# lgemc/WildlifeMapper

Measured on AMD Instinct MI355X. Metric: 1024x1024 tiles/sec (whole node), higher is better.
Workload: dtype fp16; 1 GPU; vit_h full path fft+encoder+decoder+PostProcess/NMS, fp16 MFMA, batch=16 tiles/GPU of 1024x1024x3 (BASELINE.json configs[2]); parallelism=dp1 tile shard, weights=seed 0 synthetic (random init), tolerance=logits within 1e-3 relative of the fp32 CPU forward, identical NMS index lists

## Files before the change

wildlifemapper_amd/csrc/dec_kernels.h:

```cpp
#pragma once
#include "wm_common.h"
#include "../../include/wm_hip.h"

namespace wm {

template <int HD, int QB, int NW = 1>
__global__ __launch_bounds__(64 * NW) void mha32_kernel(const float* __restrict__ q, const float* __restrict__ k,
                                                   const float* __restrict__ v, float* __restrict__ out,
                                                   int nq, int nk, int heads) {
    const int lane = threadIdx.x & 63, wave = threadIdx.x >> 6;
    const int q0 = blockIdx.x * QB, head = blockIdx.y, b = blockIdx.z;
    const int C = heads * HD;
    const float scale = 1.0f / sqrtf((float)HD);
    float qv[QB][HD], m[QB], l[QB], acc[QB][HD];
#pragma unroll
    for (int i = 0; i < QB; ++i) {
        const int qi = min(q0 + i, nq - 1);
        const float* qp = q + ((size_t)b * nq + qi) * C + head * HD;
#pragma unroll
        for (int d = 0; d < HD; d += 4) {
            const f32x4 t = *(const f32x4*)(qp + d);
            qv[i][d] = t[0]; qv[i][d + 1] = t[1]; qv[i][d + 2] = t[2]; qv[i][d + 3] = t[3];
        }
        m[i] = -1e30f; l[i] = 0.f;
#pragma unroll
        for (int d = 0; d < HD; ++d) acc[i][d] = 0.f;
    }
    for (int key = wave * 64 + lane; key < nk; key += 64 * NW) {
        const float* kp = k + ((size_t)b * nk + key) * C + head * HD;
        const float* vp = v + ((size_t)b * nk + key) * C + head * HD;
        float kr[HD], vr[HD];
#pragma unroll
        for (int d = 0; d < HD; d += 4) {
            const f32x4 t = *(const f32x4*)(kp + d);
// ... 269 lines not shown
            if (sscore[j] > score || (sscore[j] == score && j < i)) ++rank;
        }
    }
    if (cand) sorder[rank] = i;
    __syncthreads();
    int nms_rank = -1, kept = 0;
    for (int r = 0; r < ncand; ++r) {
        const int a = sorder[r];
        const bool alive = sdead[a] == 0;
        if (alive) {
            if (i == a) nms_rank = kept;
            ++kept;
            if (cand && rank > r && sdead[i] == 0) {
                const float xx0 = fmaxf(sx0[a], x0), yy0 = fmaxf(sy0[a], y0);
                const float xx1 = fminf(sx1[a], x1), yy1 = fminf(sy1[a], y1);
                const float iw = fmaxf(0.f, xx1 - xx0), ih = fmaxf(0.f, yy1 - yy0);
                const float inter = iw * ih;
                const float iou = inter / (sarea[a] + sarea[i] - inter);
                if (iou > iou_thr) sdead[i] = 1;
            }
        }
        __syncthreads();
    }
    if (live) {
        wm_box_record o;
        o.box[0] = x0; o.box[1] = y0; o.box[2] = x1; o.box[3] = y1;
        o.score = score; o.label = label;
        o.flags = (conf ? WM_FLAG_CONF : 0) | (cand ? WM_FLAG_SCORE : 0) | (nms_rank >= 0 ? WM_FLAG_NMS : 0);
        o.nms_rank = nms_rank;
        rec[(size_t)b * NQ + i] = o;
    }
}

__global__ __launch_bounds__(256) void add_bcast_kernel(const float* __restrict__ a, const float* __restrict__ b, float* __restrict__ out,
                                                        int64_t rows, int C, int mod) {
    const int64_t n4 = rows * C / 4;
    for (int64_t i = (int64_t)blockIdx.x * 256 + threadIdx.x; i < n4; i += (int64_t)gridDim.x * 256) {
        const int64_t r = (i * 4) / C;
        const int c = (int)((i * 4) % C);
        const f32x4 y = *(const f32x4*)(b + (r % mod) * C + c);
        *(f32x4*)(out + i * 4) = a ? *(const f32x4*)(a + i * 4) + y : y;
    }
}

}
```

wildlifemapper_amd/csrc/host_attn.h:

```cpp
#pragma once
#include "attn_glob4.h"
#include "attn_glob8.h"
#include "attn_window.h"
#include "dec_kernels.h"
#include "misc_kernels.h"
#include "host_core.h"

namespace {

struct AttnTimeline { const char* tag = nullptr; int waves = 0, marks = 0; };
template <auto KERN, class... Extra>
int launch_attn(wm_handle* h, hipStream_t s, int kclass, double flops, AttnTimeline tl, int grid, int block, int lds, const AttnArgs& a, Extra... extra) {
    lds += (tl.tag && WM_DEV_TIMELINE) ? 4096 : 0;
    WM_TRY(set_max_lds((const void*)KERN, lds));
    Bracket br(h, s, kclass, flops, 0.0);
    if (tl.tag) WM_DEV_HOOK((dev_attn_timeline<KERN>(tl.tag, tl.waves, tl.marks, dim3(grid), dim3(block), lds, s, a, extra...)));
    hipLaunchKernelGGL(KERN, dim3(grid), dim3(block), lds, s, a, extra...);
    HIP_TRY(hipGetLastError());
    return 0;
}

template <class T16, int HD, bool REL>
int launch_attn_global_t(wm_handle* h, hipStream_t s, const AttnArgs& a, int batch, int kclass) {
    static const bool four_wave = getenv("WM_ATTN_4WAVE") && atoi(getenv("WM_ATTN_4WAVE")) != 0;
    const double flops = 4.0 * batch * a.heads * (double)a.nq * a.nk * HD;
    if (a.nq % 256 == 0 && a.nk >= 128 && !four_wave)
        return launch_attn<attn_global8_kernel<T16, HD, REL>>(h, s, kclass, flops, {"g8", 8, 64}, (a.nq / 256) * a.heads * batch, 512, Global8Lds<HD, REL>::TOTAL, a);
    return launch_attn<attn_global_kernel<T16, HD, REL>>(h, s, kclass, flops, {}, (a.nq / 128) * a.heads * batch, 256, GlobalLds<HD, REL>::TOTAL, a);
}

template <class T16>
int launch_attn_global_p(wm_handle* h, hipStream_t s, const AttnArgs& a, int batch, int hd, bool rel, int kclass) {
    if (a.nq % 128 || a.nk % 64) return fail("attention: nq=%d nk=%d must be multiples of 128/64", a.nq, a.nk);
    if (rel && (a.nq != T || a.nk != T)) return fail("attention: rel-pos path needs 4096 queries and keys");
    auto none = [&] { return fail("attention: head_dim=%d rel=%d not built (64, 80, 128)", hd, (int)rel); };
    if (rel) return by_head_dim<64, 80>(hd, [&](auto d) { return launch_attn_global_t<T16, decltype(d)::value, true>(h, s, a, batch, kclass); }, none);
    return by_head_dim<64, 80, 128>(hd, [&](auto d) { return launch_attn_global_t<T16, decltype(d)::value, false>(h, s, a, batch, kclass); }, none);
}
int launch_attn_global(wm_handle* h, hipStream_t s, int prec, const AttnArgs& a, int batch, int hd, bool rel) {
// ... 51 lines not shown
    if (!x.q_prescaled) WM_TRY(scale_q_copy(s, prec, a, batch, D));
    if (window == 0) return launch_attn_global(h, s, prec, a, batch, hd, true);
    if (window != 14) return fail("attention: window=%d unsupported (14 or 0)", window);
    {
        uint16_t* b16 = nullptr;
        bool convert = true;
        if (h) {
            auto it = h->bias16.find({qkv_bias, prec});
            if (it != h->bias16.end()) { b16 = it->second; convert = false; }
            else { WM_TRY(dalloc(h, &b16, (size_t)3 * D * 2)); h->bias16[{qkv_bias, prec}] = b16; }
        } else {
            void* pb = nullptr;
            WM_TRY(op_scratch(s, 0, (size_t)3 * D * 2, &pb));
            b16 = (uint16_t*)pb;
        }
        if (convert) WM_TRY(launch_cvt_f32_to_16(s, prec, qkv_bias, b16, 3 * D / 4));
        a.qkv_bias16 = (const u16*)b16;
    }
    return by_head_dim<64, 80>(hd, [&](auto d) {
        return by_type16(prec, [&](auto t) { return launch_attn_window_t<decltype(t), decltype(d)::value>(h, s, a, batch); });
    }, [&] { return fail("attention: head_dim=%d not built for windows (64, 80)", hd); });
}

int launch_mha16(wm_handle* h, hipStream_t s, int prec, const void* q, int qs, const void* k, int ks, const void* v, int vs,
                 void* out, int os, int batch, int heads, int hd, int nq, int nk, int q_prescaled = 0) {
    AttnArgs a{};
    a.q = (const u16*)q; a.k = (const u16*)k; a.v = (const u16*)v; a.out = (u16*)out;
    a.q_stride = qs; a.k_stride = ks; a.v_stride = vs; a.out_stride = os;
    a.nq = nq; a.nk = nk; a.scale = 1.0f / sqrtf((float)hd); a.heads = heads;
    if (!q_prescaled) WM_TRY(scale_q_copy(s, prec, a, batch, heads * hd));
    return launch_attn_global(h, s, prec, a, batch, hd, false);
}

int launch_mha32(wm_handle* h, hipStream_t s, const float* q, const float* k, const float* v, float* out, int batch,
                 int heads, int hd, int nq, int nk) {
    Bracket br(h, s, WM_KCLASS_OTHER, 4.0 * batch * heads * (double)nq * nk * hd, 0.0);
    const bool share = nk >= 1024;
    constexpr int KC = 256;
    if (hd == 16 && nq <= 64 && nk >= 1024 && nk % KC == 0) {
        const int nchunk = nk / KC;
        const size_t need = (size_t)batch * heads * nchunk * 64 * (16 + 2) * 4;
        float* part = nullptr;
        if (h) {
            if (h->mha_part_cap < need) {
                if (h->mha_part) dfree(h, h->mha_part);
                h->mha_part = nullptr; h->mha_part_cap = 0;
                WM_TRY(dalloc(h, &h->mha_part, need));
                h->mha_part_cap = need;
            }
            part = h->mha_part;
        } else {
            void* pb = nullptr;
            WM_TRY(op_scratch(s, 1, need, &pb));
            part = (float*)pb;
        }
        hipLaunchKernelGGL((mha32_keysplit_kernel<16, KC>), dim3(nchunk, heads, batch), dim3(256), 0, s, q, k, v, part, nq, nk, heads);
        hipLaunchKernelGGL((mha32_merge_chunks_kernel<16>), dim3(heads, batch), dim3(64 * 4), 0, s, (const float*)part, out, nq, nchunk, heads);
    } else if (hd == 16 && nk == NQ && nq >= 1024)
        hipLaunchKernelGGL((mha32_fewkeys_kernel<16, NQ>), dim3((nq + 255) / 256, heads, batch), dim3(256), 0, s, q, k, v, out, nq, heads);
    else if (hd == 16 && share) hipLaunchKernelGGL((mha32_kernel<16, 4, 4>), dim3((nq + 3) / 4, heads, batch), dim3(256), 0, s, q, k, v, out, nq, nk, heads);
    else if (hd == 16) hipLaunchKernelGGL((mha32_kernel<16, 1>), dim3(nq, heads, batch), dim3(64), 0, s, q, k, v, out, nq, nk, heads);
    else if (hd == 32) hipLaunchKernelGGL((mha32_kernel<32, 1>), dim3(nq, heads, batch), dim3(64), 0, s, q, k, v, out, nq, nk, heads);
    else return fail("mha32: head_dim=%d not built (16, 32)", hd);
    HIP_TRY(hipGetLastError());
    return 0;
}

}
```

wildlifemapper_amd/csrc/host_core.h:

```cpp
#pragma once
#include <hip/hip_runtime.h>

#include <cmath>
#include <cstdarg>
#include <cstdio>
#include <cstdlib>
#include <cstring>
#include <atomic>
#include <map>
#include <tuple>
#include <type_traits>
#include <mutex>
#include <set>
#include <string>
#include <algorithm>
#include <array>
#include <vector>

#include "../../include/wm_hip.h"
#include "wm_common.h"

#ifndef WM_DEV_TIMELINE
#define WM_DEV_TIMELINE 0
#endif
// ... 125 lines not shown
    hipEvent_t a, b;
    int kclass;
    double flops, bytes;
};

struct Profiler {
    bool on = false;
    std::vector<EvPair> used;
    std::vector<std::pair<hipEvent_t, hipEvent_t>> pool;
    wm_kclass_stat acc[WM_KCLASS_COUNT] = {};
};

}

struct wm_handle {
    wm_config cfg{};
    int fp8_gemms = WM_FP8_ALL;
    int fp8_bf16_tail = 0, fp8_bf16_head = 0;
    int fp16_tail = 0;
    int device = 0;
    int D = 0, depth = 0, heads = 0, hd = 0, prec = 0, maxB = 0;
    bool is_global[64] = {};
    bool finalized = false, enc_ready = false, dec_ready = false;
    std::map<std::string, std::vector<int64_t>> expected;
    std::map<std::string, HostW> staged;
    std::map<std::string, uint16_t*> w16;
    std::map<std::string, uint16_t*> wfold;
    std::map<std::string, float*> fold_c1, fold_c2;
    std::map<std::string, float*> wsrc32;
    float* fold_stats = nullptr;
    uint16_t* lo16 = nullptr;
    bool split = false;
    bool rows8 = true;
    bool fold_from16 = false;
    int* overflow = nullptr;
    bool fold = false, fold_bf16 = false;
    std::map<std::string, uint16_t*> w16p;
    std::map<std::string, uint8_t*> w8k;
    std::map<std::string, uint8_t*> w8;
    uint8_t* ao8 = nullptr;
    std::map<std::string, float*> w32;
    std::vector<void*> allocs;
    Profiler prof;
    std::map<const float*, std::pair<uint16_t*, uint16_t*>> w32x3;
    std::map<std::pair<const float*, int>, uint16_t*> bias16;
    float* mha_part = nullptr;
    size_t mha_part_cap = 0;
    bool row_major = false;
    bool sat_on = false;
    unsigned long long* sat_counts = nullptr;
    int tap_which = -2;
    float* tap_buf = nullptr;

    float *resid = nullptr, *tokbase = nullptr;
    uint16_t *xn16 = nullptr, *ao16 = nullptr, *qkv16 = nullptr, *hid16 = nullptr;
    uint16_t *p16 = nullptr, *h16 = nullptr, *he16 = nullptr, *hp16 = nullptr, *pt16 = nullptr, *q16 = nullptr,
             *kv16 = nullptr, *aoh16 = nullptr, *y1n16 = nullptr, *h1_16 = nullptr, *y2_16 = nullptr, *y2t16 = nullptr;
    float *pt32 = nullptr, *y1 = nullptr, *y1n32 = nullptr, *z32 = nullptr;
    float *n1 = nullptr, *n2 = nullptr, *emb_nhwc = nullptr, *emb_nchw = nullptr;
    uint16_t *n1n16 = nullptr, *x16last = nullptr;
    float *dkeys = nullptr, *dk_a = nullptr, *dk_b = nullptr, *dk_c = nullptr;
    float *dq = nullptr, *dt_q = nullptr, *dt_k = nullptr, *dt_v = nullptr, *dt_att = nullptr, *dt_hid = nullptr,
          *dt_h1 = nullptr, *dt_h2 = nullptr;
    float *logits = nullptr, *boxes = nullptr, *hfc = nullptr, *tsz_default = nullptr;
    float2 *fftR = nullptr, *fft_tw = nullptr;
    float* kpe = nullptr;
// ... 82 lines not shown
```

wildlifemapper_amd/csrc/host_decoder.h:

```cpp
#pragma once
#include "dec_kernels.h"
#include "host_encoder.h"

namespace {

struct DecAttnW { const float *wq, *bq, *wk, *bk, *wv, *bv, *wo, *bo; int internal; };

DecAttnW dec_w(wm_handle* h, const std::string& p, int internal) {
    return DecAttnW{W32(h, p + "q_proj.weight"), W32(h, p + "q_proj.bias"), W32(h, p + "k_proj.weight"), W32(h, p + "k_proj.bias"),
                    W32(h, p + "v_proj.weight"), W32(h, p + "v_proj.bias"), W32(h, p + "out_proj.weight"), W32(h, p + "out_proj.bias"), internal};
}

int decoder_impl(wm_handle* h, const float* keys_nhwc, float* logits, float* boxes, int B, hipStream_t s) {
    const std::string t = "mask_decoder.transformer.";
    const int E = OUTC, Mk = B * T, Mq = B * NQ;
    const float* tok = W32(h, "mask_decoder.mask_tokens.weight");
    float* keys = h->dkeys;
    HIP_TRY(hipMemcpyAsync(keys, keys_nhwc, (size_t)Mk * E * 4, hipMemcpyDeviceToDevice, s));
    float* queries = h->dq;
    WM_TRY(launch_simple(h, s, 0.0, add_bcast_kernel, dim3(grid_for((int64_t)Mq * E / 4)), dim3(256), (const float*)nullptr, tok, queries, (int64_t)Mq, E, NQ));

    auto add_q = [&](float* out) {
        return launch_simple(h, s, 0.0, add_bcast_kernel, dim3(grid_for((int64_t)Mq * E / 4)), dim3(256), (const float*)queries, tok, out, (int64_t)Mq, E, NQ);
    };
    auto add_k = [&](float* out) {
        return launch_simple(h, s, 0.0, add_bcast_kernel, dim3(grid_for((int64_t)Mk * E / 4)), dim3(256), (const float*)keys, (const float*)h->kpe, out, (int64_t)Mk, E, T);
    };
    auto ln = [&](float* x, const std::string& n, int rows) {
        return launch_layernorm(h, s, WM_PREC_FP16, x, W32(h, n + ".weight"), W32(h, n + ".bias"), 1e-5f, x, nullptr, rows, E);
    };
    auto token_to_image = [&](const DecAttnW& w, const float* kin) -> int {
        WM_TRY(add_q(h->dt_h1));
        WM_TRY(launch_gemm32(h, s, h->dt_h1, w.wq, w.bq, nullptr, h->dt_q, Mq, w.internal, E, ACT_NONE));
        WM_TRY(launch_gemm32(h, s, kin, w.wk, w.bk, nullptr, h->dk_a, Mk, w.internal, E, ACT_NONE));
        WM_TRY(launch_gemm32(h, s, keys, w.wv, w.bv, nullptr, h->dk_b, Mk, w.internal, E, ACT_NONE));
        WM_TRY(launch_mha32(h, s, h->dt_q, h->dk_a, h->dk_b, h->dt_att, B, 8, w.internal / 8, NQ, T));
        WM_TRY(launch_gemm32(h, s, h->dt_att, w.wo, w.bo, queries, queries, Mq, E, w.internal, ACT_NONE));
        return 0;
    };
    float* kpe_sum = h->n1;

    for (int i = 0; i < 2; ++i) {
        const std::string L = t + "layers." + std::to_string(i) + ".";
        {
            const DecAttnW w = dec_w(h, L + "self_attn.", E);
            const float* qin = queries;
            if (i != 0) { WM_TRY(add_q(h->dt_h1)); qin = h->dt_h1; }
            WM_TRY(launch_gemm32(h, s, qin, w.wq, w.bq, nullptr, h->dt_q, Mq, E, E, ACT_NONE));
            WM_TRY(launch_gemm32(h, s, qin, w.wk, w.bk, nullptr, h->dt_k, Mq, E, E, ACT_NONE));
            WM_TRY(launch_gemm32(h, s, queries, w.wv, w.bv, nullptr, h->dt_v, Mq, E, E, ACT_NONE));
            WM_TRY(launch_mha32(h, s, h->dt_q, h->dt_k, h->dt_v, h->dt_att, B, 8, E / 8, NQ, NQ));
            WM_TRY(launch_gemm32(h, s, h->dt_att, w.wo, w.bo, i == 0 ? nullptr : queries, queries, Mq, E, E, ACT_NONE));
            WM_TRY(ln(queries, L + "norm1", Mq));
        }
        WM_TRY(add_k(kpe_sum));
        WM_TRY(token_to_image(dec_w(h, L + "cross_attn_token_to_image.", E / 2), kpe_sum));
        WM_TRY(ln(queries, L + "norm2", Mq));
        WM_TRY(launch_gemm32(h, s, queries, W32(h, L + "mlp.lin1.weight"), W32(h, L + "mlp.lin1.bias"), nullptr, h->dt_hid, Mq, DEC_MLP, E, ACT_RELU));
        WM_TRY(launch_gemm32(h, s, h->dt_hid, W32(h, L + "mlp.lin2.weight"), W32(h, L + "mlp.lin2.bias"), queries, queries, Mq, E, DEC_MLP, ACT_NONE));
        WM_TRY(ln(queries, L + "norm3", Mq));
        {
            const DecAttnW w = dec_w(h, L + "cross_attn_image_to_token.", E / 2);
            WM_TRY(add_q(h->dt_h1));
            WM_TRY(launch_gemm32(h, s, kpe_sum, w.wq, w.bq, nullptr, h->dk_a, Mk, w.internal, E, ACT_NONE));
            WM_TRY(launch_gemm32(h, s, h->dt_h1, w.wk, w.bk, nullptr, h->dt_k, Mq, w.internal, E, ACT_NONE));
            WM_TRY(launch_gemm32(h, s, queries, w.wv, w.bv, nullptr, h->dt_v, Mq, w.internal, E, ACT_NONE));
            WM_TRY(launch_mha32(h, s, h->dk_a, h->dt_k, h->dt_v, h->dk_c, B, 8, w.internal / 8, T, NQ));
            WM_TRY(launch_gemm32(h, s, h->dk_c, w.wo, w.bo, keys, keys, Mk, E, w.internal, ACT_NONE));
            WM_TRY(ln(keys, L + "norm4", Mk));
        }
    }
    WM_TRY(add_k(kpe_sum));
    WM_TRY(token_to_image(dec_w(h, t + "final_attn_token_to_image.", E / 2), kpe_sum));
    WM_TRY(ln(queries, t + "norm_final_attn", Mq));

    const std::string c = "mask_decoder.class_embed.layers.", bb = "mask_decoder.bbox_embed.layers.";
    WM_TRY(launch_gemm32(h, s, queries, W32(h, c + "0.weight"), W32(h, c + "0.bias"), nullptr, h->dt_h1, Mq, E, E, ACT_RELU));
    WM_TRY(launch_gemm32(h, s, h->dt_h1, W32(h, c + "1.weight"), W32(h, c + "1.bias"), nullptr, h->dt_h2, Mq, E, E, ACT_RELU));
    WM_TRY(launch_gemm32(h, s, h->dt_h2, W32(h, c + "2.weight"), W32(h, c + "2.bias"), nullptr, logits, Mq, WM_NUM_LOGITS, E, ACT_NONE));
    WM_TRY(launch_gemm32(h, s, queries, W32(h, bb + "0.weight"), W32(h, bb + "0.bias"), nullptr, h->dt_h1, Mq, E, E, ACT_RELU));
    WM_TRY(launch_gemm32(h, s, h->dt_h1, W32(h, bb + "1.weight"), W32(h, bb + "1.bias"), nullptr, h->dt_h2, Mq, E, E, ACT_RELU));
    WM_TRY(launch_gemm32(h, s, h->dt_h2, W32(h, bb + "2.weight"), W32(h, bb + "2.bias"), nullptr, boxes, Mq, 4, E, ACT_SIGMOID));
    return 0;
}

int forward_impl(wm_handle* h, const float* x_dev, const float* target_sizes_dev, float* logits_dev, float* boxes_dev,
                 wm_box_record* records_dev, int batch, hipStream_t s) {
    WM_TRY(fft_impl(h, x_dev, h->hfc, batch, s, true));
    WM_TRY(encoder_impl(h, x_dev, h->hfc, nullptr, batch, s, true));
    WM_TRY(decoder_impl(h, h->emb_nhwc, h->logits, h->boxes, batch, s));
    const float* ts = target_sizes_dev ? target_sizes_dev : h->tsz_default;
    WM_TRY(launch_simple(h, s, 0.0, postprocess_nms_kernel, dim3(batch), dim3(64), (const float*)h->logits, (const float*)h->boxes, ts,
                         0.05f, 0.5f, 0.4f, h->records));
    if (logits_dev) HIP_TRY(hipMemcpyAsync(logits_dev, h->logits, (size_t)batch * NQ * WM_NUM_LOGITS * 4, hipMemcpyDeviceToDevice, s));
    if (boxes_dev) HIP_TRY(hipMemcpyAsync(boxes_dev, h->boxes, (size_t)batch * NQ * 16, hipMemcpyDeviceToDevice, s));
    if (records_dev) HIP_TRY(hipMemcpyAsync(records_dev, h->records, (size_t)batch * NQ * sizeof(wm_box_record), hipMemcpyDeviceToDevice, s));
    return 0;
}

}
```

wildlifemapper_amd/csrc/host_gemm.h:

```cpp
#pragma once
#include "gemm16.h"
#include "gemm16_v2.h"
#include "gemm16_v3.h"
#include "gemm16_v5.h"
#include "gemm32.h"
#include "gemm8.h"
#include "misc_kernels.h"
#include "host_core.h"

namespace {

double gemm16_flops(const Gemm16Args& a) { return 2.0 * a.M * (double)a.N * a.K; }
double gemm16_bytes(const Gemm16Args& a) {
    return 2.0 * ((double)a.M * a.K + (double)a.N * a.K) + (a.out32 ? 4.0 : 0.0) * a.M * a.N + (a.out16 ? 2.0 : 0.0) * a.M * a.N +
           (a.residual ? 4.0 * (double)(a.res_mod > 0 ? a.res_mod : a.M) * a.N : 0.0);
}

template <class Kern, class Args>
int launch_gemm_kernel(wm_handle* h, hipStream_t s, Kern kern, int grid, int threads, int lds, const Args& a, int variant, double flops, double bytes) {
    WM_TRY(set_max_lds((const void*)kern, lds));
    if (variant >= 0) count_variant(variant);
    Bracket br(h, s, WM_KCLASS_GEMM16, flops, bytes);
    hipLaunchKernelGGL(kern, dim3(grid), dim3(threads), lds, s, a);
    HIP_TRY(hipGetLastError());
// ... 150 lines not shown
    if (M % 4096 || N % 256 || Cin % 32) return fail("conv3x3: M=%d N=%d C=%d unsupported (M %% 4096, N %% 256, C %% 32)", M, N, Cin);
    const uint16_t* zero_page = nullptr;
    WM_TRY(zero_page_for_device(&zero_page));
    Gemm16Args a{};
    a.A = (const u16*)A; a.W = (const u16*)W; a.out32 = out32; a.M = M; a.N = N; a.K = 9 * Cin; a.act = ACT_NONE; a.conv_c = Cin; a.zero_page = (const u16*)zero_page;
    using G = G3<256>;
    count_variant(WM_GEMM_V3_CONV3X3);
    return by_type16(prec, [&](auto t) {
        return launch_gemm_kernel(h, s, gemm16v3_kernel<decltype(t), 256, ALoad::Conv3x3>, (M / 256) * (N / 256), G::THREADS, G::LDS, a, -1,
                                  2.0 * M * (double)N * 9 * Cin, 2.0 * ((double)M * Cin + 9.0 * N * Cin) + 4.0 * M * N);
    });
}

int launch_patch_embed16(wm_handle* h, hipStream_t s, int prec, const void* img16, const void* W, const float* bias, const float* res, int res_mod,
                         float* out32, void* out16, int B, int N, int Cin) {
    const int M = B * 4096, K = Cin * 256;
    if (B <= 0 || (N % 320 && N % 256) || Cin <= 0) return fail("patch_embed: B=%d N=%d Cin=%d unsupported (N %% 320 or N %% 256)", B, N, Cin);
    if (!out32 && !out16) return fail("patch_embed: no output");
    Gemm16Args a{};
    a.A = (const u16*)img16; a.W = (const u16*)W; a.bias = bias; a.residual = res; a.out32 = out32; a.out16 = (u16*)out16;
    a.M = M; a.N = N; a.K = K; a.res_mod = res_mod; a.act = ACT_NONE; a.conv_c = Cin;
    count_variant(WM_GEMM_V3_PATCH);
    const double bytes = 2.0 * ((double)M * K + (double)N * K) + (out32 ? 4.0 : 0.0) * M * N + (out16 ? 2.0 : 0.0) * M * N;
    return by_type16(prec, [&](auto t) {
        return by_tile_width(N, [&](auto bn) {
            constexpr int BN = decltype(bn)::value;
            using G = G3<BN>;
            return launch_gemm_kernel(h, s, gemm16v3_kernel<decltype(t), BN, ALoad::PatchEmbed>, (M / 256) * (N / BN), G::THREADS, G::LDS, a, -1,
                                      2.0 * M * (double)N * K, bytes);
        });
    });
}

int launch_gemm32(wm_handle* h, hipStream_t s, const float* A, const float* W, const float* bias, const float* res,
                  float* out, int M, int N, int K, int act, int lda = 0, int mode = 0) {
    if (K % 16) return fail("gemm32: K=%d must be a multiple of 16", K);
    static const bool f32_only = getenv("WM_GEMM32_F32") && atoi(getenv("WM_GEMM32_F32")) != 0;
    if ((mode == 2 || mode == 3) && K % 32) return fail("gemm32 (split form): K=%d must be a multiple of 32", K);
    if (mode == 2 || mode == 3 || (mode == 0 && h && !f32_only && K % 32 == 0)) {
        Gemm32x3Args a{A, W, nullptr, nullptr, bias, res, out, M, N, K, act, lda > 0 ? lda : K, h ? h->overflow + 1 : nullptr};
        if (mode == 3) {
            const size_t n = (size_t)N * K;
            void* pb = nullptr;
            WM_TRY(op_scratch(s, 3, n * 4, &pb));
            u16* hi = (u16*)pb;
            hipLaunchKernelGGL(split_w32_kernel, dim3(grid_for((int64_t)n / 4)), dim3(256), 0, s, W, hi, hi + n, (int64_t)n / 4, (int*)nullptr);
            HIP_TRY(hipGetLastError());
            a.Whi = hi; a.Wlo = hi + n;
        }
        if (mode == 0) {
            auto it = h->w32x3.find(W);
            if (it == h->w32x3.end()) {
                uint16_t *hi = nullptr, *lo = nullptr;
                const size_t n = (size_t)N * K;
                if (n % 4) return fail("gemm32: weight of %zu elements", n);
                WM_TRY(dalloc(h, &hi, n * 2)); WM_TRY(dalloc(h, &lo, n * 2));
                hipLaunchKernelGGL(split_w32_kernel, dim3(grid_for((int64_t)n / 4)), dim3(256), 0, s, W, (u16*)hi, (u16*)lo, (int64_t)n / 4, h->overflow + 1);
                HIP_TRY(hipGetLastError());
                it = h->w32x3.emplace(W, std::make_pair(hi, lo)).first;
            }
            a.Whi = (const u16*)it->second.first; a.Wlo = (const u16*)it->second.second;
        }
        Bracket br(h, s, WM_KCLASS_OTHER, 2.0 * M * (double)N * K, 4.0 * ((double)M * K + (double)M * N) + 4.0 * (double)N * K);
        const dim3 grid(((N + 63) / 64) * ((M + 63) / 64));
        if (mode == 0 || mode == 3) hipLaunchKernelGGL(gemm32x3_kernel<true>, grid, dim3(256), 0, s, a);
        else hipLaunchKernelGGL(gemm32x3_kernel<false>, grid, dim3(256), 0, s, a);
        HIP_TRY(hipGetLastError());
        return 0;
    }
    Gemm32Args a{A, W, bias, res, out, M, N, K, act, lda > 0 ? lda : K};
    Bracket br(h, s, WM_KCLASS_OTHER, 2.0 * M * (double)N * K, 4.0 * ((double)M * K + (double)N * K + (double)M * N));
    hipLaunchKernelGGL(gemm32_kernel, dim3(((N + 63) / 64) * ((M + 63) / 64)), dim3(256), 0, s, a);
    HIP_TRY(hipGetLastError());
    return 0;
}

}
```

wildlifemapper_amd/csrc/host_weights.h:

```cpp
#pragma once
#include "misc_kernels.h"
#include "fft_kernels.h"
#include "host_core.h"

namespace {

bool ends_with(const std::string& s, const char* suf) {
    const size_t n = strlen(suf);
    return s.size() >= n && s.compare(s.size() - n, n, suf) == 0;
}

static inline uint16_t f32_to_bf16_host(float f) {
    uint32_t u;
    memcpy(&u, &f, 4);
    if ((u & 0x7fffffffu) > 0x7f800000u) return (uint16_t)((u >> 16) | 0x40);
    u += 0x7fffu + ((u >> 16) & 1u);
    return (uint16_t)(u >> 16);
}

static inline uint16_t f32_to_f16_host(float f) {
    _Float16 h = (_Float16)fminf(fmaxf(f, -65504.f), 65504.f);
    uint16_t r;
    memcpy(&r, &h, 2);
    return r;
// ... 183 lines not shown
    WM_TRY(dalloc(h, &d, n * 4));
    HIP_TRY(hipMemcpy(d, src, n * 4, hipMemcpyHostToDevice));
    h->w32[key] = d;
    return 0;
}

const uint16_t* W16(wm_handle* h, const std::string& n) { return h->w16.at(n); }
const uint16_t* W16P(wm_handle* h, const std::string& n) {
    if (h->row_major) return nullptr;
    auto it = h->w16p.find(n);
    return it == h->w16p.end() ? nullptr : it->second;
}
const float* W32(wm_handle* h, const std::string& n) { return h->w32.at(n); }

int launch_fold_weight(hipStream_t s, int prec, const void* w16, const float* w32, const float* g, const float* be, const float* bias, void* wf,
                       float* c1, float* c2, int N, int K) {
    return by_type16(prec, [&](auto t) {
        return launch_simple(nullptr, s, 0.0, fold_weight_kernel<decltype(t)>, dim3(N), dim3(256), (const u16*)w16, w32, g, be, bias, (u16*)wf, c1, c2, N, K);
    });
}

int create_impl(const wm_config* cfg, int device, wm_handle** out) {
    HIP_TRY(hipSetDevice(device));
    wm_handle* h = new wm_handle();
    h->cfg = *cfg; h->device = device;
    h->fp16_tail = getenv("WM_FP16_TAIL") ? atoi(getenv("WM_FP16_TAIL")) : 0;
    h->fp8_bf16_tail = getenv("WM_FP8_BF16_TAIL") ? atoi(getenv("WM_FP8_BF16_TAIL")) : 0;
    h->fp8_bf16_head = getenv("WM_FP8_BF16_HEAD") ? atoi(getenv("WM_FP8_BF16_HEAD")) : 0;
    h->row_major = getenv("WM_ROW_MAJOR_OPERANDS") && atoi(getenv("WM_ROW_MAJOR_OPERANDS")) != 0;
    h->fold = (cfg->flags & (WM_CFG_FOLD_LN | WM_CFG_FOLD_LN_BF16)) != 0 && !h->row_major;
    h->fold_bf16 = (cfg->flags & WM_CFG_FOLD_LN_BF16) != 0;
    h->fold_from16 = getenv("WM_FOLD_FROM16") && atoi(getenv("WM_FOLD_FROM16")) != 0;
    h->rows8 = !(getenv("WM_FP8_ROWS") && atoi(getenv("WM_FP8_ROWS")) == 0);
    h->split = h->fold && !(getenv("WM_STREAM_SPLIT") && atoi(getenv("WM_STREAM_SPLIT")) == 0);
    h->fp8_gemms = cfg->fp8_gemms ? (cfg->fp8_gemms & WM_FP8_ALL) : (getenv("WM_FP8_GEMMS") ? (atoi(getenv("WM_FP8_GEMMS")) & WM_FP8_ALL) : WM_FP8_ALL);
    if (cfg->precision == WM_PREC_FP8 && h->fp8_gemms == 0) { delete h; return fail("wm_create: fp8_gemms selects no GEMM"); }
    h->D = cfg->embed_dim; h->depth = cfg->depth; h->heads = cfg->num_heads; h->hd = cfg->embed_dim / cfg->num_heads;
    h->prec = cfg->precision; h->maxB = cfg->max_batch;
    for (int i = 0; i < cfg->num_global; ++i) {
        const int g = cfg->global_attn_indexes[i];
        if (g < 0 || g >= cfg->depth) { delete h; return fail("wm_create: global index %d out of range", g); }
        h->is_global[g] = true;
    }
    build_expected(h);

    const size_t B = (size_t)h->maxB, D = (size_t)h->D, BT = B * T;
    int r = 0;
#define A(ptr, bytes) if (!r) r = dalloc(h, &h->ptr, (bytes))
    A(resid, BT * D * 4); A(tokbase, BT * D * 4);
    A(xn16, BT * D * 2); A(ao16, BT * D * 2); A(qkv16, BT * 3 * D * 2); A(hid16, BT * 4 * D * 2);
    A(p16, BT * 768 * 2); A(h16, BT * 256 * 2); A(he16, BT * HFC * 2); A(hp16, BT * HFC * 2); A(pt16, BT * HFC * 2);
    A(q16, BT * HFC * 2); A(kv16, BT * 2 * HFC * 2); A(aoh16, BT * HFC * 2); A(y1n16, BT * HFC * 2); A(h1_16, BT * HFC * 2);
    A(y2_16, BT * HFC * 2); A(y2t16, BT * HFC * 2);
    A(pt32, BT * HFC * 4); A(y1, BT * HFC * 4); A(y1n32, BT * HFC * 4); A(z32, BT * HFC * 4);
    A(n1, BT * OUTC * 4); A(n2, BT * OUTC * 4); A(emb_nhwc, BT * OUTC * 4); A(emb_nchw, BT * OUTC * 4);
    A(n1n16, BT * OUTC * 2); A(x16last, BT * D * 2);
    if (cfg->precision == WM_PREC_FP8) { A(ao8, BT * D); }
    A(dkeys, BT * OUTC * 4); A(dk_a, BT * 128 * 4); A(dk_b, BT * 128 * 4); A(dk_c, BT * 128 * 4);
    A(dq, B * NQ * OUTC * 4); A(dt_q, B * NQ * OUTC * 4); A(dt_k, B * NQ * OUTC * 4); A(dt_v, B * NQ * OUTC * 4);
    A(dt_att, B * NQ * OUTC * 4); A(dt_hid, B * NQ * DEC_MLP * 4); A(dt_h1, B * NQ * OUTC * 4); A(dt_h2, B * NQ * OUTC * 4);
    A(logits, B * NQ * WM_NUM_LOGITS * 4); A(boxes, B * NQ * 4 * 4);
    A(hfc, B * 1024 * 1024 * 4); A(tsz_default, B * 2 * 4);
    A(fftR, B * FFT_N * FFT_L * sizeof(float2)); A(fft_tw, FFT_N * sizeof(float2));
    A(kpe, (size_t)T * OUTC * 4);
    A(records, B * NQ * sizeof(wm_box_record));
    A(sat_counts, WM_SAT_COUNT * sizeof(unsigned long long));
// ... 156 lines not shown
```

Measured before the change: 169.6 tiles/s.

## Fuse decoder cross-attention K/V projections with attention and output LayerNorm

Adds two fused kernels for the two-way transformer decoder. The token-to-image kernel adds the positional encoding, runs the K and V projections with split fp16 hi/lo MFMA, and does the online-softmax attention per chunk, writing partials that a merge kernel combines. The image-to-token kernel fuses the Q projection, attention over the query tokens, the output projection, the residual add and LayerNorm. This removes the large per-token K/V/Q intermediates, the kpe add passes and the keys copy, at the cost of more complex kernels with high LDS use and a chunked partial merge.

```diff
diff --git a/wildlifemapper_amd/csrc/dec_kernels.h b/wildlifemapper_amd/csrc/dec_kernels.h
--- a/wildlifemapper_amd/csrc/dec_kernels.h
+++ b/wildlifemapper_amd/csrc/dec_kernels.h
@@ -1,5 +1,6 @@
 #pragma once
 #include "wm_common.h"
+#include "gemm32.h"
 #include "../../include/wm_hip.h"
 
 namespace wm {
@@ -335,6 +336,320 @@
     }
 }
 
+constexpr int DF_BM = 64;
+constexpr int DF_E = 256, DF_I = 128;
+constexpr int DF_LDA = DF_E + 8, DF_LDI = DF_I + 8;
+constexpr int DF_PLANE = DF_BM * DF_LDA;
+constexpr int DF_KC = 256;
+static_assert(WM_NUM_QUERIES <= 64, "lane = query");
+
+__device__ __forceinline__ void df_split8(const f32x4& x0, const f32x4& x1, float& amax, uint4& hi, uint4& lo) {
+    union { uint4 raw; typename FP16::vec4 h[2]; } uh, ul;
+#pragma unroll
+    for (int j = 0; j < 8; ++j) {
+        const float x = j < 4 ? x0[j] : x1[j - 4];
+        amax = fmaxf(amax, fabsf(x));
+        uh.h[j >> 2][j & 3] = FP16::from_f32_bounded(x);
+        ul.h[j >> 2][j & 3] = FP16::from_f32_bounded((x - FP16::to_f32(uh.h[j >> 2][j & 3])) * G32X3_LOSCALE);
+    }
+    hi = uh.raw; lo = ul.raw;
+}
+
+template <int K, int RT, int UNR = K / 16>
+__device__ __forceinline__ void df_mma(const u16* sAh, const u16* sAl, int lda, const u16* __restrict__ Whi, const u16* __restrict__ Wlo,
+                                       int n0, int lane, f32x16 (&acc)[RT], f32x16 (&accx)[RT]) {
+    const size_t wo = (size_t)(n0 + (lane & 31)) * K + 8 * (lane >> 5);
+    const int fa = (lane & 31) * lda + 8 * (lane >> 5);
+#pragma unroll
+    for (int rt = 0; rt < RT; ++rt)
+#pragma unroll
+        for (int r = 0; r < 16; ++r) acc[rt][r] = accx[rt][r] = 0.f;
+#pragma unroll UNR
+    for (int ks = 0; ks < K / 16; ++ks) {
+        const typename FP16::vec8 w_hi = *(const typename FP16::vec8*)(Whi + wo + 16 * ks), w_lo = *(const typename FP16::vec8*)(Wlo + wo + 16 * ks);
+#pragma unroll
+        for (int rt = 0; rt < RT; ++rt) {
+            const typename FP16::vec8 a_hi = *(const typename FP16::vec8*)(sAh + fa + rt * 32 * lda + 16 * ks);
+            const typename FP16::vec8 a_lo = *(const typename FP16::vec8*)(sAl + fa + rt * 32 * lda + 16 * ks);
+            accx[rt] = FP16::mfma32(a_lo, w_hi, accx[rt]);
+            accx[rt] = FP16::mfma32(a_hi, w_lo, accx[rt]);
+            acc[rt] = FP16::mfma32(a_hi, w_hi, acc[rt]);
+        }
+    }
+}
+__device__ __forceinline__ int df_row(int r, int lane) { return (r & 3) + 8 * (r >> 2) + 4 * (lane >> 5); }
+__device__ __forceinline__ float df_val(float a, float ax, float bias) { return (a + ax * (1.0f / G32X3_LOSCALE)) * (1.0f / G32X3_WSCALE) + bias; }
+
+struct DecT2IArgs {
+    const float* keys; const float* pe;
+    const u16 *wk_hi, *wk_lo, *wv_hi, *wv_lo;
+    const float *bk, *bv;
+    const float* q;
+    float* part;
+    int* overflow;
+};
+constexpr int DF_T2I_LDS = 4 * DF_PLANE * 2;
+
+__global__ __launch_bounds__(512) void dec_token_to_image_kernel(DecT2IArgs p) {
+    constexpr int HD = 16, NQ = WM_NUM_QUERIES, NT = 512, NU = DF_BM * DF_E / 8 / NT, NSB = DF_KC / DF_BM;
+    extern __shared__ __attribute__((aligned(16))) char smem[];
+    u16* P1h = (u16*)smem; u16* P1l = P1h + DF_PLANE; u16* P2h = P1l + DF_PLANE; u16* P2l = P2h + DF_PLANE;
+    float* sK = (float*)P1h; float* sV = (float*)P2h;
+    static_assert(DF_BM * DF_I * 4 <= 2 * DF_PLANE * 2, "k / v over their planes");
+    const int tid = threadIdx.x, lane = tid & 63;
+    const int wave = __builtin_amdgcn_readfirstlane(tid >> 6);
+    const int chunk = blockIdx.x, b = blockIdx.y, nchunk = gridDim.x;
+    const float* kb = p.keys + ((size_t)b * 4096 + (size_t)chunk * DF_KC) * DF_E;
+    const float* pb = p.pe + (size_t)chunk * DF_KC * DF_E;
+    f32x4 xk[NU][2], xp[NU][2];
+    auto fetch = [&](int sb) {
+#pragma unroll
+        for (int i = 0; i < NU; ++i) {
+            const int u = tid + i * NT, off = (sb * DF_BM + (u >> 5)) * DF_E + (u & 31) * 8;
+            xk[i][0] = *(const f32x4*)(kb + off); xk[i][1] = *(const f32x4*)(kb + off + 4);
+            xp[i][0] = *(const f32x4*)(pb + off); xp[i][1] = *(const f32x4*)(pb + off + 4);
+        }
+    };
+    fetch(0);
+    const int head = wave;
+    float qv[HD], acc[HD];
+    {
+        const float scale = 1.44269504088896340736f / sqrtf((float)HD);
+        const float* qp = p.q + ((size_t)b * NQ + min(lane, NQ - 1)) * DF_I + head * HD;
+#pragma unroll
+        for (int d = 0; d < HD; d += 4) {
+            const f32x4 t = *(const f32x4*)(qp + d);
+            qv[d] = t[0] * scale; qv[d + 1] = t[1] * scale; qv[d + 2] = t[2] * scale; qv[d + 3] = t[3] * scale;
+        }
+    }
+    float m = -1e30f, l = 0.f, amax = 0.f;
+#pragma unroll
+    for (int d = 0; d < HD; ++d) acc[d] = 0.f;
+    const bool isv = wave >= 4;
+    const int n0 = (wave & 3) * 32;
+    const float bias = (isv ? p.bv : p.bk)[n0 + (lane & 31)];
+
+    for (int sb = 0; sb < NSB; ++sb) {
+#pragma unroll
+        for (int i = 0; i < NU; ++i) {
+            const int u = tid + i * NT, o = (u >> 5) * DF_LDA + (u & 31) * 8;
+            uint4 hi, lo;
+            df_split8(xk[i][0] + xp[i][0], xk[i][1] + xp[i][1], amax, hi, lo);
+            *(uint4*)(P1h + o) = hi; *(uint4*)(P1l + o) = lo;
+            df_split8(xk[i][0], xk[i][1], amax, hi, lo);
+            *(uint4*)(P2h + o) = hi; *(uint4*)(P2l + o) = lo;
+        }
+        __syncthreads();
+        f32x16 c[2], cx[2];
+        df_mma<DF_E, 2, 8>(isv ? P2h : P1h, isv ? P2l : P1l, DF_LDA, isv ? p.wv_hi : p.wk_hi, isv ? p.wv_lo : p.wk_lo, n0, lane, c, cx);
+        __syncthreads();
+        {
+            float* dst = (isv ? sV : sK) + n0 + (lane & 31);
+#pragma unroll
+            for (int rt = 0; rt < 2; ++rt)
+#pragma unroll
+                for (int r = 0; r < 16; ++r) dst[(rt * 32 + df_row(r, lane)) * DF_I] = df_val(c[rt][r], cx[rt][r], bias);
+        }
+        if (sb + 1 < NSB) fetch(sb + 1);
+        __syncthreads();
+        constexpr int KB = 8;
+        for (int j0 = 0; j0 < DF_BM; j0 += KB) {
+            float sc[KB];
+            float bm = -1e30f;
+#pragma unroll
+            for (int j = 0; j < KB; ++j) {
+                const float* kr = sK + (j0 + j) * DF_I + head * HD;
+                float t0 = 0.f;
+#pragma unroll
+                for (int d = 0; d < HD; d += 4) {
+                    const f32x4 t = *(const f32x4*)(kr + d);
+                    t0 = fmaf(qv[d], t[0], t0); t0 = fmaf(qv[d + 1], t[1], t0); t0 = fmaf(qv[d + 2], t[2], t0); t0 = fmaf(qv[d + 3], t[3], t0);
+                }
+                sc[j] = t0;
+                bm = fmaxf(bm, t0);
+            }
+            const float mn = fmaxf(m, bm);
+            const float a = __builtin_amdgcn_exp2f(m - mn);
+            l *= a;
+#pragma unroll
+            for (int d = 0; d < HD; ++d) acc[d] *= a;
+            m = mn;
+#pragma unroll
+            for (int j = 0; j < KB; ++j) {
+                const float* vr = sV + (j0 + j) * DF_I + head * HD;
+                const float pe = __builtin_amdgcn_exp2f(sc[j] - mn);
+                l += pe;
+#pragma unroll
+                for (int d = 0; d < HD; d += 4) {
+                    const f32x4 u = *(const f32x4*)(vr + d);
+                    acc[d] = fmaf(pe, u[0], acc[d]); acc[d + 1] = fmaf(pe, u[1], acc[d + 1]);
+                    acc[d + 2] = fmaf(pe, u[2], acc[d + 2]); acc[d + 3] = fmaf(pe, u[3], acc[d + 3]);
+                }
+            }
+        }
+        __syncthreads();
+    }
+    if (lane < NQ) {
+        float* dst = p.part + ((((size_t)b * 8 + head) * nchunk + chunk) * 64 + lane) * (HD + 2);
+#pragma unroll
+        for (int d = 0; d < HD; ++d) dst[d] = acc[d];
+        dst[HD] = m; dst[HD + 1] = l;
+    }
+    if (amax >= 65504.f && p.overflow) *(volatile int*)p.overflow = 1;
+}
+
+struct DecI2TArgs {
+    const float* kin; float* kout; const float* pe;
+    const u16 *wq_hi, *wq_lo; const float* bq;
+    const float *tk, *tv;
+    const u16 *wo_hi, *wo_lo; const float* bo;
+    const float *gamma, *beta; float eps;
+    int* overflow;
+};
+constexpr int DF_LDQ = DF_I + 4, DF_LDY = DF_E + 4;
+constexpr int DF_I2T_ATT = DF_BM * DF_LDQ * 4;
+constexpr int DF_I2T_LDS = DF_I2T_ATT + 2 * DF_BM * DF_LDI * 2;
+static_assert(DF_I2T_LDS >= 2 * DF_PLANE * 2 && DF_I2T_LDS >= DF_BM * DF_LDY * 4, "one region, three uses");
+
+__global__ __launch_bounds__(256, 2) void dec_image_to_token_kernel(DecI2TArgs p) {
+    constexpr int HD = 16, NK = WM_NUM_QUERIES, NT = 256, NU = DF_BM * DF_E / 8 / NT, HALF = NU / 2;
+    extern __shared__ __attribute__((aligned(16))) char smem[];
+    u16* Ph = (u16*)smem; u16* Pl = Ph + DF_PLANE;
+    float* sQ = (float*)smem;
+    u16* Ah = (u16*)(smem + DF_I2T_ATT); u16* Al = Ah + DF_BM * DF_LDI;
+    float* sY = (float*)smem;
+    const int tid = threadIdx.x, lane = tid & 63;
+    const int wave = __builtin_amdgcn_readfirstlane(tid >> 6);
+    const size_t row0 = (size_t)blockIdx.x * DF_BM;
+    const int b = (int)(row0 / 4096), t0 = (int)(row0 % 4096);
+    const float* kb = p.kin + row0 * DF_E;
+    const float* pb = p.pe + (size_t)t0 * DF_E;
+    float amax = 0.f;
+#pragma unroll
+    for (int hf = 0; hf < 2; ++hf) {
+        f32x4 xk[HALF][2], xp[HALF][2];
+#pragma unroll
+        for (int i = 0; i < HALF; ++i) {
+            const int u = tid + (hf * HALF + i) * NT, off = (u >> 5) * DF_E + (u & 31) * 8;
+            xk[i][0] = *(const f32x4*)(kb + off); xk[i][1] = *(const f32x4*)(kb + off + 4);
+            xp[i][0] = *(const f32x4*)(pb + off); xp[i][1] = *(const f32x4*)(pb + off + 4);
+        }
+#pragma unroll
+        for (int i = 0; i < HALF; ++i) {
+            const int u = tid + (hf * HALF + i) * NT, o = (u >> 5) * DF_LDA + (u & 31) * 8;
+            uint4 hi, lo;
+            df_split8(xk[i][0] + xp[i][0], xk[i][1] + xp[i][1], amax, hi, lo);
+            *(uint4*)(Ph + o) = hi; *(uint4*)(Pl + o) = lo;
+        }
+    }
+    __syncthreads();
+    {
+        f32x16 c[2], cx[2];
+        const int n = wave * 32 + (lane & 31);
+        df_mma<DF_E, 2>(Ph, Pl, DF_LDA, p.wq_hi, p.wq_lo, wave * 32, lane, c, cx);
+        const float bias = p.bq[n];
+        __syncthreads();
+#pragma unroll
+        for (int rt = 0; rt < 2; ++rt)
+#pragma unroll
+            for (int r = 0; r < 16; ++r) sQ[(rt * 32 + df_row(r, lane)) * DF_LDQ + n] = df_val(c[rt][r], cx[rt][r], bias);
+    }
+    __syncthreads();
+#pragma unroll 1
+    for (int hh = 0; hh < 2; ++hh) {
+        const int head = wave * 2 + hh;
+        const float scale = 1.44269504088896340736f / sqrtf((float)HD);
+        float qv[HD];
+#pragma unroll
+        for (int d = 0; d < HD; d += 4) {
+            const f32x4 t = *(const f32x4*)(sQ + lane * DF_LDQ + head * HD + d);
+            qv[d] = t[0] * scale; qv[d + 1] = t[1] * scale; qv[d + 2] = t[2] * scale; qv[d + 3] = t[3] * scale;
+        }
+        const float* __restrict__ tk = p.tk + (size_t)b * NK * DF_I + head * HD;
+        const float* __restrict__ tv = p.tv + (size_t)b * NK * DF_I + head * HD;
+        constexpr int KB = 3;
+        static_assert(NK % KB == 0, "key blocks");
+        float m = -1e30f, l = 0.f, acc[HD];
+#pragma unroll
+        for (int d = 0; d < HD; ++d) acc[d] = 0.f;
+#pragma unroll 1
+        for (int j0 = 0; j0 < NK; j0 += KB) {
+            float sc[KB];
+            float bm = -1e30f;
+#pragma unroll
+            for (int j = 0; j < KB; ++j) {
+                float t0 = 0.f;
+#pragma unroll
+                for (int d = 0; d < HD; ++d) t0 = fmaf(qv[d], tk[(j0 + j) * DF_I + d], t0);
+                sc[j] = t0;
+                bm = fmaxf(bm, t0);
+            }
+            const float mn = fmaxf(m, bm);
+            const float a = __builtin_amdgcn_exp2f(m - mn);
+            l *= a;
+#pragma unroll
+            for (int d = 0; d < HD; ++d) acc[d] *= a;
+            m = mn;
+#pragma unroll
+            for (int j = 0; j < KB; ++j) {
+                const float pe = __builtin_amdgcn_exp2f(sc[j] - mn);
+                l += pe;
+#pragma unroll
+                for (int d = 0; d < HD; ++d) acc[d] = fmaf(pe, tv[(j0 + j) * DF_I + d], acc[d]);
+            }
+        }
+        const float inv = 1.0f / l;
+#pragma unroll
+        for (int d = 0; d < HD; d += 8) {
+            uint4 hi, lo;
+            df_split8(f32x4{acc[d] * inv, acc[d + 1] * inv, acc[d + 2] * inv, acc[d + 3] * inv},
+                      f32x4{acc[d + 4] * inv, acc[d + 5] * inv, acc[d + 6] * inv, acc[d + 7] * inv}, amax, hi, lo);
+            *(uint4*)(Ah + lane * DF_LDI + head * HD + d) = hi; *(uint4*)(Al + lane * DF_LDI + head * HD + d) = lo;
+        }
+    }
+    __syncthreads();
+    {
+        f32x16 c[2][2], cx[2][2];
+#pragma unroll
+        for (int ct = 0; ct < 2; ++ct) df_mma<DF_I, 2>(Ah, Al, DF_LDI, p.wo_hi, p.wo_lo, wave * 64 + ct * 32, lane, c[ct], cx[ct]);
+        __syncthreads();
+#pragma unroll
+        for (int ct = 0; ct < 2; ++ct) {
+            const int n = wave * 64 + ct * 32 + (lane & 31);
+            const float bias = p.bo[n];
+#pragma unroll
+            for (int rt = 0; rt < 2; ++rt)
+#pragma unroll
+                for (int r = 0; r < 16; ++r) {
+                    const int mr = rt * 32 + df_row(r, lane);
+                    sY[mr * DF_LDY + n] = df_val(c[ct][rt][r], cx[ct][rt][r], bias) + kb[(size_t)mr * DF_E + n];
+                }
+        }
+    }
+    __syncthreads();
+    {
+        const f32x4 g = *(const f32x4*)(p.gamma + lane * 4), be = *(const f32x4*)(p.beta + lane * 4);
+        for (int i = 0; i < DF_BM / 4; ++i) {
+            const int r = wave * (DF_BM / 4) + i;
+            const f32x4 v = *(const f32x4*)(sY + r * DF_LDY + lane * 4);
+            const float mean = wave_sum((v[0] + v[1]) + (v[2] + v[3])) * (1.0f / DF_E);
+            float sq = 0.f;
+#pragma unroll
+            for (int j = 0; j < 4; ++j) {
+                const float d = v[j] - mean;
+                sq += d * d;
+            }
+            const float var = wave_sum(sq) * (1.0f / DF_E);
+            const float rstd = 1.0f / sqrtf(var + p.eps);
+            f32x4 y;
+#pragma unroll
+            for (int j = 0; j < 4; ++j) y[j] = (v[j] - mean) * rstd * g[j] + be[j];
+            *(f32x4*)(p.kout + (row0 + r) * DF_E + lane * 4) = y;
+        }
+    }
+    if (amax >= 65504.f && p.overflow) *(volatile int*)p.overflow = 1;
+}
+
 __global__ __launch_bounds__(256) void add_bcast_kernel(const float* __restrict__ a, const float* __restrict__ b, float* __restrict__ out,
                                                         int64_t rows, int C, int mod) {
     const int64_t n4 = rows * C / 4;
diff --git a/wildlifemapper_amd/csrc/host_attn.h b/wildlifemapper_amd/csrc/host_attn.h
--- a/wildlifemapper_amd/csrc/host_attn.h
+++ b/wildlifemapper_amd/csrc/host_attn.h
@@ -5,6 +5,7 @@
 #include "dec_kernels.h"
 #include "misc_kernels.h"
 #include "host_core.h"
+#include "host_gemm.h"
 
 namespace {
 
@@ -122,6 +123,59 @@
     return launch_attn_global(h, s, prec, a, batch, hd, false);
 }
 
+int mha32_partials(wm_handle* h, hipStream_t s, int batch, int heads, int nchunk, float** part) {
+    const size_t need = (size_t)batch * heads * nchunk * 64 * (16 + 2) * 4;
+    if (h) {
+        if (h->mha_part_cap < need) {
+            if (h->mha_part) dfree(h, h->mha_part);
+            h->mha_part = nullptr; h->mha_part_cap = 0;
+            WM_TRY(dalloc(h, &h->mha_part, need));
+            h->mha_part_cap = need;
+        }
+        *part = h->mha_part;
+    } else {
+        void* pb = nullptr;
+        WM_TRY(op_scratch(s, 1, need, &pb));
+        *part = (float*)pb;
+    }
+    return 0;
+}
+
+int launch_dec_token_to_image(wm_handle* h, hipStream_t s, const float* keys, const float* q, const float* wk, const float* bk,
+                              const float* wv, const float* bv, float* out, int batch) {
+    DecT2IArgs a{};
+    a.keys = keys; a.pe = h->kpe; a.bk = bk; a.bv = bv; a.q = q; a.overflow = h->overflow + 1;
+    WM_TRY(gemm32_w_planes(h, s, wk, DF_I, DF_E, &a.wk_hi, &a.wk_lo));
+    WM_TRY(gemm32_w_planes(h, s, wv, DF_I, DF_E, &a.wv_hi, &a.wv_lo));
+    constexpr int nchunk = T / DF_KC, heads = 8;
+    WM_TRY(mha32_partials(h, s, batch, heads, nchunk, &a.part));
+    WM_TRY(set_max_lds((const void*)dec_token_to_image_kernel, DF_T2I_LDS));
+    const double rows = (double)batch * T;
+    Bracket br(h, s, WM_KCLASS_OTHER, 2.0 * rows * 2 * DF_I * DF_E + 4.0 * batch * heads * (double)NQ * T * 16,
+               4.0 * rows * DF_E + 4.0 * T * DF_E + 2.0 * 4 * DF_I * DF_E + 2.0 * 4 * batch * heads * nchunk * 64 * 18);
+    hipLaunchKernelGGL(dec_token_to_image_kernel, dim3(nchunk, batch), dim3(512), DF_T2I_LDS, s, a);
+    hipLaunchKernelGGL((mha32_merge_chunks_kernel<16>), dim3(heads, batch), dim3(64 * 4), 0, s, (const float*)a.part, out, NQ, nchunk, heads);
+    HIP_TRY(hipGetLastError());
+    return 0;
+}
+
+int launch_dec_image_to_token(wm_handle* h, hipStream_t s, const float* kin, float* kout, const float* wq, const float* bq,
+                              const float* tk, const float* tv, const float* wo, const float* bo, const float* gamma, const float* beta,
+                              int batch) {
+    DecI2TArgs a{};
+    a.kin = kin; a.kout = kout; a.pe = h->kpe; a.bq = bq; a.tk = tk; a.tv = tv; a.bo = bo; a.gamma = gamma; a.beta = beta; a.eps = 1e-5f;
+    a.overflow = h->overflow + 1;
+    WM_TRY(gemm32_w_planes(h, s, wq, DF_I, DF_E, &a.wq_hi, &a.wq_lo));
+    WM_TRY(gemm32_w_planes(h, s, wo, DF_E, DF_I, &a.wo_hi, &a.wo_lo));
+    WM_TRY(set_max_lds((const void*)dec_image_to_token_kernel, DF_I2T_LDS));
+    const double rows = (double)batch * T;
+    Bracket br(h, s, WM_KCLASS_OTHER, 2.0 * rows * 2 * DF_I * DF_E + 4.0 * rows * 8 * (double)NQ * 16,
+               2 * 4.0 * rows * DF_E + 4.0 * T * DF_E + 2.0 * 4 * DF_I * DF_E + 2 * 4.0 * batch * NQ * DF_I);
+    hipLaunchKernelGGL(dec_image_to_token_kernel, dim3(batch * (T / DF_BM)), dim3(256), DF_I2T_LDS, s, a);
+    HIP_TRY(hipGetLastError());
+    return 0;
+}
+
 int launch_mha32(wm_handle* h, hipStream_t s, const float* q, const float* k, const float* v, float* out, int batch,
                  int heads, int hd, int nq, int nk) {
     Bracket br(h, s, WM_KCLASS_OTHER, 4.0 * batch * heads * (double)nq * nk * hd, 0.0);
@@ -129,21 +183,8 @@
     constexpr int KC = 256;
     if (hd == 16 && nq <= 64 && nk >= 1024 && nk % KC == 0) {
         const int nchunk = nk / KC;
-        const size_t need = (size_t)batch * heads * nchunk * 64 * (16 + 2) * 4;
         float* part = nullptr;
-        if (h) {
-            if (h->mha_part_cap < need) {
-                if (h->mha_part) dfree(h, h->mha_part);
-                h->mha_part = nullptr; h->mha_part_cap = 0;
-                WM_TRY(dalloc(h, &h->mha_part, need));
-                h->mha_part_cap = need;
-            }
-            part = h->mha_part;
-        } else {
-            void* pb = nullptr;
-            WM_TRY(op_scratch(s, 1, need, &pb));
-            part = (float*)pb;
-        }
+        WM_TRY(mha32_partials(h, s, batch, heads, nchunk, &part));
         hipLaunchKernelGGL((mha32_keysplit_kernel<16, KC>), dim3(nchunk, heads, batch), dim3(256), 0, s, q, k, v, part, nq, nk, heads);
         hipLaunchKernelGGL((mha32_merge_chunks_kernel<16>), dim3(heads, batch), dim3(64 * 4), 0, s, (const float*)part, out, nq, nchunk, heads);
     } else if (hd == 16 && nk == NQ && nq >= 1024)
diff --git a/wildlifemapper_amd/csrc/host_core.h b/wildlifemapper_amd/csrc/host_core.h
--- a/wildlifemapper_amd/csrc/host_core.h
+++ b/wildlifemapper_amd/csrc/host_core.h
@@ -181,6 +181,7 @@
     uint16_t* lo16 = nullptr;
     bool split = false;
     bool rows8 = true;
+    bool dec_fuse = true;
     bool fold_from16 = false;
     int* overflow = nullptr;
     bool fold = false, fold_bf16 = false;
diff --git a/wildlifemapper_amd/csrc/host_decoder.h b/wildlifemapper_amd/csrc/host_decoder.h
--- a/wildlifemapper_amd/csrc/host_decoder.h
+++ b/wildlifemapper_amd/csrc/host_decoder.h
@@ -16,7 +16,10 @@
     const int E = OUTC, Mk = B * T, Mq = B * NQ;
     const float* tok = W32(h, "mask_decoder.mask_tokens.weight");
     float* keys = h->dkeys;
-    HIP_TRY(hipMemcpyAsync(keys, keys_nhwc, (size_t)Mk * E * 4, hipMemcpyDeviceToDevice, s));
+    const bool fuse = h->dec_fuse && !gemm32_f32_only();
+    const float* kcur = keys;
+    if (fuse) kcur = keys_nhwc;
+    else HIP_TRY(hipMemcpyAsync(keys, keys_nhwc, (size_t)Mk * E * 4, hipMemcpyDeviceToDevice, s));
     float* queries = h->dq;
     WM_TRY(launch_simple(h, s, 0.0, add_bcast_kernel, dim3(grid_for((int64_t)Mq * E / 4)), dim3(256), (const float*)nullptr, tok, queries, (int64_t)Mq, E, NQ));
 
@@ -32,9 +35,12 @@
     auto token_to_image = [&](const DecAttnW& w, const float* kin) -> int {
         WM_TRY(add_q(h->dt_h1));
         WM_TRY(launch_gemm32(h, s, h->dt_h1, w.wq, w.bq, nullptr, h->dt_q, Mq, w.internal, E, ACT_NONE));
-        WM_TRY(launch_gemm32(h, s, kin, w.wk, w.bk, nullptr, h->dk_a, Mk, w.internal, E, ACT_NONE));
-        WM_TRY(launch_gemm32(h, s, keys, w.wv, w.bv, nullptr, h->dk_b, Mk, w.internal, E, ACT_NONE));
-        WM_TRY(launch_mha32(h, s, h->dt_q, h->dk_a, h->dk_b, h->dt_att, B, 8, w.internal / 8, NQ, T));
+        if (fuse) WM_TRY(launch_dec_token_to_image(h, s, kcur, h->dt_q, w.wk, w.bk, w.wv, w.bv, h->dt_att, B));
+        else {
+            WM_TRY(launch_gemm32(h, s, kin, w.wk, w.bk, nullptr, h->dk_a, Mk, w.internal, E, ACT_NONE));
+            WM_TRY(launch_gemm32(h, s, keys, w.wv, w.bv, nullptr, h->dk_b, Mk, w.internal, E, ACT_NONE));
+            WM_TRY(launch_mha32(h, s, h->dt_q, h->dk_a, h->dk_b, h->dt_att, B, 8, w.internal / 8, NQ, T));
+        }
         WM_TRY(launch_gemm32(h, s, h->dt_att, w.wo, w.bo, queries, queries, Mq, E, w.internal, ACT_NONE));
         return 0;
     };
@@ -53,7 +59,7 @@
             WM_TRY(launch_gemm32(h, s, h->dt_att, w.wo, w.bo, i == 0 ? nullptr : queries, queries, Mq, E, E, ACT_NONE));
             WM_TRY(ln(queries, L + "norm1", Mq));
         }
-        WM_TRY(add_k(kpe_sum));
+        if (!fuse) WM_TRY(add_k(kpe_sum));
         WM_TRY(token_to_image(dec_w(h, L + "cross_attn_token_to_image.", E / 2), kpe_sum));
         WM_TRY(ln(queries, L + "norm2", Mq));
         WM_TRY(launch_gemm32(h, s, queries, W32(h, L + "mlp.lin1.weight"), W32(h, L + "mlp.lin1.bias"), nullptr, h->dt_hid, Mq, DEC_MLP, E, ACT_RELU));
@@ -62,15 +68,21 @@
         {
             const DecAttnW w = dec_w(h, L + "cross_attn_image_to_token.", E / 2);
             WM_TRY(add_q(h->dt_h1));
-            WM_TRY(launch_gemm32(h, s, kpe_sum, w.wq, w.bq, nullptr, h->dk_a, Mk, w.internal, E, ACT_NONE));
             WM_TRY(launch_gemm32(h, s, h->dt_h1, w.wk, w.bk, nullptr, h->dt_k, Mq, w.internal, E, ACT_NONE));
             WM_TRY(launch_gemm32(h, s, queries, w.wv, w.bv, nullptr, h->dt_v, Mq, w.internal, E, ACT_NONE));
-            WM_TRY(launch_mha32(h, s, h->dk_a, h->dt_k, h->dt_v, h->dk_c, B, 8, w.internal / 8, T, NQ));
-            WM_TRY(launch_gemm32(h, s, h->dk_c, w.wo, w.bo, keys, keys, Mk, E, w.internal, ACT_NONE));
-            WM_TRY(ln(keys, L + "norm4", Mk));
+            if (fuse) {
+                WM_TRY(launch_dec_image_to_token(h, s, kcur, keys, w.wq, w.bq, h->dt_k, h->dt_v, w.wo, w.bo, W32(h, L + "norm4.weight"),
+                                                 W32(h, L + "norm4.bias"), B));
+                kcur = keys;
+            } else {
+                WM_TRY(launch_gemm32(h, s, kpe_sum, w.wq, w.bq, nullptr, h->dk_a, Mk, w.internal, E, ACT_NONE));
+                WM_TRY(launch_mha32(h, s, h->dk_a, h->dt_k, h->dt_v, h->dk_c, B, 8, w.internal / 8, T, NQ));
+                WM_TRY(launch_gemm32(h, s, h->dk_c, w.wo, w.bo, keys, keys, Mk, E, w.internal, ACT_NONE));
+                WM_TRY(ln(keys, L + "norm4", Mk));
+            }
         }
     }
-    WM_TRY(add_k(kpe_sum));
+    if (!fuse) WM_TRY(add_k(kpe_sum));
     WM_TRY(token_to_image(dec_w(h, t + "final_attn_token_to_image.", E / 2), kpe_sum));
     WM_TRY(ln(queries, t + "norm_final_attn", Mq));
 
diff --git a/wildlifemapper_amd/csrc/host_gemm.h b/wildlifemapper_amd/csrc/host_gemm.h
--- a/wildlifemapper_amd/csrc/host_gemm.h
+++ b/wildlifemapper_amd/csrc/host_gemm.h
@@ -206,10 +206,30 @@
     });
 }
 
+bool gemm32_f32_only() {
+    static const bool f32_only = getenv("WM_GEMM32_F32") && atoi(getenv("WM_GEMM32_F32")) != 0;
+    return f32_only;
+}
+
+int gemm32_w_planes(wm_handle* h, hipStream_t s, const float* W, int N, int K, const u16** hi_out, const u16** lo_out) {
+    auto it = h->w32x3.find(W);
+    if (it == h->w32x3.end()) {
+        uint16_t *hi = nullptr, *lo = nullptr;
+        const size_t n = (size_t)N * K;
+        if (n % 4) return fail("gemm32: weight of %zu elements", n);
+        WM_TRY(dalloc(h, &hi, n * 2)); WM_TRY(dalloc(h, &lo, n * 2));
+        hipLaunchKernelGGL(split_w32_kernel, dim3(grid_for((int64_t)n / 4)), dim3(256), 0, s, W, (u16*)hi, (u16*)lo, (int64_t)n / 4, h->overflow + 1);
+        HIP_TRY(hipGetLastError());
+        it = h->w32x3.emplace(W, std::make_pair(hi, lo)).first;
+    }
+    *hi_out = (const u16*)it->second.first; *lo_out = (const u16*)it->second.second;
+    return 0;
+}
+
 int launch_gemm32(wm_handle* h, hipStream_t s, const float* A, const float* W, const float* bias, const float* res,
                   float* out, int M, int N, int K, int act, int lda = 0, int mode = 0) {
     if (K % 16) return fail("gemm32: K=%d must be a multiple of 16", K);
-    static const bool f32_only = getenv("WM_GEMM32_F32") && atoi(getenv("WM_GEMM32_F32")) != 0;
+    const bool f32_only = gemm32_f32_only();
     if ((mode == 2 || mode == 3) && K % 32) return fail("gemm32 (split form): K=%d must be a multiple of 32", K);
     if (mode == 2 || mode == 3 || (mode == 0 && h && !f32_only && K % 32 == 0)) {
         Gemm32x3Args a{A, W, nullptr, nullptr, bias, res, out, M, N, K, act, lda > 0 ? lda : K, h ? h->overflow + 1 : nullptr};
@@ -222,19 +242,7 @@
             HIP_TRY(hipGetLastError());
             a.Whi = hi; a.Wlo = hi + n;
         }
-        if (mode == 0) {
-            auto it = h->w32x3.find(W);
-            if (it == h->w32x3.end()) {
-                uint16_t *hi = nullptr, *lo = nullptr;
-                const size_t n = (size_t)N * K;
-                if (n % 4) return fail("gemm32: weight of %zu elements", n);
-                WM_TRY(dalloc(h, &hi, n * 2)); WM_TRY(dalloc(h, &lo, n * 2));
-                hipLaunchKernelGGL(split_w32_kernel, dim3(grid_for((int64_t)n / 4)), dim3(256), 0, s, W, (u16*)hi, (u16*)lo, (int64_t)n / 4, h->overflow + 1);
-                HIP_TRY(hipGetLastError());
-                it = h->w32x3.emplace(W, std::make_pair(hi, lo)).first;
-            }
-            a.Whi = (const u16*)it->second.first; a.Wlo = (const u16*)it->second.second;
-        }
+        if (mode == 0) WM_TRY(gemm32_w_planes(h, s, W, N, K, &a.Whi, &a.Wlo));
         Bracket br(h, s, WM_KCLASS_OTHER, 2.0 * M * (double)N * K, 4.0 * ((double)M * K + (double)M * N) + 4.0 * (double)N * K);
         const dim3 grid(((N + 63) / 64) * ((M + 63) / 64));
         if (mode == 0 || mode == 3) hipLaunchKernelGGL(gemm32x3_kernel<true>, grid, dim3(256), 0, s, a);
diff --git a/wildlifemapper_amd/csrc/host_weights.h b/wildlifemapper_amd/csrc/host_weights.h
--- a/wildlifemapper_amd/csrc/host_weights.h
+++ b/wildlifemapper_amd/csrc/host_weights.h
@@ -239,6 +239,7 @@
     h->fold_bf16 = (cfg->flags & WM_CFG_FOLD_LN_BF16) != 0;
     h->fold_from16 = getenv("WM_FOLD_FROM16") && atoi(getenv("WM_FOLD_FROM16")) != 0;
     h->rows8 = !(getenv("WM_FP8_ROWS") && atoi(getenv("WM_FP8_ROWS")) == 0);
+    h->dec_fuse = !(getenv("WM_DEC_FUSE") && atoi(getenv("WM_DEC_FUSE")) == 0);
     h->split = h->fold && !(getenv("WM_STREAM_SPLIT") && atoi(getenv("WM_STREAM_SPLIT")) == 0);
     h->fp8_gemms = cfg->fp8_gemms ? (cfg->fp8_gemms & WM_FP8_ALL) : (getenv("WM_FP8_GEMMS") ? (atoi(getenv("WM_FP8_GEMMS")) & WM_FP8_ALL) : WM_FP8_ALL);
     if (cfg->precision == WM_PREC_FP8 && h->fp8_gemms == 0) { delete h; return fail("wm_create: fp8_gemms selects no GEMM"); }
```

Result: no change. 170.0 tiles/s, median of 6 (+0.2%).
